# EPFL-VILAB/MultiMAE

Measured on AMD Instinct MI355X. Metric: pre-train images/sec (whole node), ViT-B RGB+D+S 224^2 98-vis-tok, higher is better.
Workload: dtype bf16 (fp32_output_adapters: fp16 storage); 1 GPU; BASELINE.json configs[2]: ViT-B, RGB+depth+semseg, 224^2, Dirichlet alpha=1.0, 98 visible tokens, 4 cross-attention decoders (dim 256, depth 2), semseg adapter (fp32_output_adapters) with fp16 STORAGE (activations / saved tensors / gradients of the adapter as IEEE half in HBM: every matmul input carries the 11-bit significand TF32 gave the reference on A100; gradients stored times a power of two f; per_gpu_batch=256, global_batch=256, parallelism=dp1

## Files before the change

include/mmae.h:

```cpp
#ifndef MMAE_H
#define MMAE_H

#include <stddef.h>
#include <stdint.h>

#ifdef __cplusplus
extern "C" {
#endif

#define MMAE_ABI_VERSION 7

#define MMAE_F32  0
#define MMAE_BF16 1
#define MMAE_F32X3 2
#define MMAE_F32F16 3
#define MMAE_MXFP8 4

#define MMAE_F16 5

#define MMAE_EINVAL   (-1)
#define MMAE_ELAUNCH  (-2)
#define MMAE_ESUPPORT (-3)

int mmae_abi_version(void);
// ... 27 lines not shown
    int32_t tile;
    int32_t split_k;
    void* ws;
    int64_t ws_elems;
    float* colsum_part;
    float* a_colsum;
    int32_t a_colsum_acc;
    const void* a_scale;
    const void* b_scale;
    void* q_out; void* q_scale;
    int64_t ldq;
    const float* a_amax;
    const float* ln_gamma; const float* ln_beta; void* ln_out; float* ln_mean; float* ln_rstd; float ln_eps;
} mmae_gemm_desc;

int mmae_gemm(const mmae_gemm_desc* d, void* stream);
int mmae_gemm_plan(const mmae_gemm_desc* d, int* tile, int* split_k);
int mmae_gemm_auto_splitk(int M, int N, int K, int ab_dtype);
int mmae_gemm_cu_reserve(int k);
int mmae_gemm_cu_share(int k);
int mmae_gemm_side_cus(int k);
#ifdef MMAE_EXPERIMENTS
int mmae_gemm_duo_occupancy(int tile);
#endif

int64_t mmae_mx_scale_bytes(int rows, int cols);
int mmae_mx_quant(const void* x, int x_dtype, int64_t ldx, int rows, int cols, void* q, int64_t ldq, void* scales, void* stream);
int mmae_mx_quant_t(const void* w, int w_dtype, int64_t ldw, int n, int k, void* q, int64_t ldq, void* scales, void* stream);
int mmae_mx_quant_rows_t(const void* x, int x_dtype, int64_t ldx, int M, int C, void* q, int64_t ldq, void* scales, void* stream);
int mmae_mx_wgrad(int on);
int mmae_gelu_grad_aux(int on);
int mmae_ln_fuse(int on);
int mmae_xattn_fuse(int on);
int mmae_mx_scale_clear(void* scales, int rows, int cols, void* stream);
int mmae_layernorm_fwd_mx(const float* x, const float* gamma, const float* beta, void* y_bf16, float* mean, float* rstd, int64_t R, int D,
                          float eps, void* q, void* scales, void* stream);
int mmae_attn_fwd_mx(const void* q, const void* k, const void* v, void* o, float* lse, int B, int H, int Nq, int Nk, int hd,
                     int64_t q_sb, int64_t q_sr, int64_t k_sb, int64_t k_sr, int64_t v_sb, int64_t v_sr, int64_t o_sb, int64_t o_sr,
                     float scale, void* mx_q, void* mx_scale, void* stream);
int mmae_attn_bwd_mx(const void* q, const void* k, const void* v, const void* o, const void* d_o, const float* lse, void* dq, void* dk,
                     void* dv, int B, int H, int Nq, int Nk, int hd, int64_t q_sb, int64_t q_sr, int64_t k_sb, int64_t k_sr, int64_t v_sb,
                     int64_t v_sr, int64_t o_sb, int64_t o_sr, int64_t dq_sb, int64_t dq_sr, int64_t dk_sb, int64_t dk_sr, int64_t dv_sb,
                     int64_t dv_sr, float scale, void* mx_q, void* mx_scale, void* stream);
int64_t mmae_mx_tmp_bytes(int rows, int cols);
int mmae_mx_prepare_weights(int n, const void* const* w, int w_dtype, const int32_t* n_out, const int32_t* k_in, void* const* dst, void* stream);
int mmae_probe_mx_mfma(const int32_t* a_64x8, const int32_t* b_64x8, const int32_t* scale_a_64, const int32_t* scale_b_64, int opsel_a, int opsel_b,
                       float* out_64x16, void* stream);

int mmae_gemm_timing_enable(int on);
int mmae_gemm_timing_read(double* ms3, double* flop3, int64_t* calls3);
int mmae_gemm_timing_read_bytes(double* bytes3);

typedef struct mmae_dw_problem {
    const void* dy; int64_t ldy;
    const void* x; int64_t ldx;
    float* dw; float* db;
    int32_t n_out, k_in;
} mmae_dw_problem;

typedef struct mmae_dw_group_desc {
    int32_t n, rows, ab_dtype, accumulate, split_k;
    mmae_dw_problem p[8];
    float* ws; int64_t ws_elems;
    const float* unscale;
} mmae_dw_group_desc;

// ... 338 lines not shown
```

multimae_amd/_lib.py:

```python
from __future__ import annotations

import ctypes
import os
import re
from typing import Dict, List, Tuple

_PKG = os.path.dirname(os.path.abspath(__file__))
HEADER = os.path.join(os.path.dirname(_PKG), 'include', 'mmae.h')
LIB_PATH = os.environ.get('MMAE_LIB') or os.path.join(_PKG, 'libmmae_hip.so')

F32, BF16, F32X3, F32F16 = 0, 1, 2, 3
MXFP8 = 4
F16 = 5
U16, I32 = 6, 7
EPI_NONE, EPI_GELU, EPI_DGELU, EPI_GELU_G, EPI_MUL = 0, 1, 2, 3, 4


class GemmDesc(ctypes.Structure):
    _fields_ = [
        ('A', ctypes.c_void_p), ('B', ctypes.c_void_p), ('C', ctypes.c_void_p),
        ('ab_dtype', ctypes.c_int32), ('c_dtype', ctypes.c_int32),
        ('M', ctypes.c_int32), ('N', ctypes.c_int32), ('K', ctypes.c_int32),
        ('a_trans', ctypes.c_int32), ('b_trans', ctypes.c_int32),
        ('lda', ctypes.c_int64), ('ldb', ctypes.c_int64), ('ldc', ctypes.c_int64),
# ... 123 lines not shown
_lib = None


def declared_symbols() -> List[str]:
    return sorted(_PROTOS)


def load() -> ctypes.CDLL:
    global _lib
    if _lib is not None:
        return _lib
    if not os.path.exists(LIB_PATH):
        raise RuntimeError(
            f'{LIB_PATH} not found: the MI355X kernel library is not built. '
            'Run `python -c "import __graft_entry__ as g; g.build()"` (or `make -C multimae_amd/csrc`). '
            'multimae_amd has no CPU / PyTorch fallback by design.')
    lib = ctypes.CDLL(LIB_PATH)
    for name, (ret, argtypes) in _PROTOS.items():
        fn = getattr(lib, name)
        fn.restype = ret
        fn.argtypes = argtypes
    if lib.mmae_abi_version() != 7:
        raise RuntimeError('libmmae_hip.so ABI version mismatch')
    for which, cls in enumerate((GemmDesc, BlockDesc, StackDesc, AdapterDesc, OptDesc, PatchSrc, DwGroupDesc, ColsumJob,
                                     OptGroupsDesc)):
        if lib.mmae_struct_size(which) != ctypes.sizeof(cls):
            raise RuntimeError(f'{cls.__name__}: ctypes mirror ({ctypes.sizeof(cls)} B) != library struct ({lib.mmae_struct_size(which)} B)')
    if os.environ.get('MMAE_MX_WGRAD') is not None:
        lib.mmae_mx_wgrad(int(os.environ['MMAE_MX_WGRAD'] != '0'))
    if os.environ.get('MMAE_LN_FUSE') is not None:
        lib.mmae_ln_fuse(int(os.environ['MMAE_LN_FUSE'] != '0'))
    if os.environ.get('MMAE_XATTN_FUSE') is not None:
        lib.mmae_xattn_fuse(int(os.environ['MMAE_XATTN_FUSE'] != '0'))
    if os.environ.get('MMAE_GELU_GRAD_AUX') is not None:
        lib.mmae_gelu_grad_aux(int(os.environ['MMAE_GELU_GRAD_AUX'] != '0'))
    _lib = lib
    return lib


class KernelError(RuntimeError):
    pass


def check(rc: int, what: str) -> None:
    if rc != 0:
        msg = load().mmae_last_error()
        raise KernelError(f'{what} failed (rc={rc}): {msg.decode() if msg else "?"}')
```

multimae_amd/csrc/attention.hip:

```cpp
#include "common.h"
#include <mutex>

#define LDS_AS __attribute__((address_space(3)))
typedef __attribute__((ext_vector_type(8))) short s16x8;

namespace {

constexpr unsigned OOB = 0x80000000u;

struct AttnArgs {
    const void *q, *k, *v, *o, *d_o;
    void *out, *dq, *dk, *dv;
    float* lse;
    int B, H, Nq, Nk, nqp, nkp;
    long long q_sb, q_sr, k_sb, k_sr, v_sb, v_sr, o_sb, o_sr, dq_sb, dq_sr, dk_sb, dk_sr, dv_sb, dv_sr;
    float scale;
    unsigned char *mx_q, *mx_s;
    long long mx_rows;
    int mx_ld, mx_col[3];
    const float* dy_amax;
};

template <int HD> __device__ __forceinline__ int tile_off(int row, int c);
template <> __device__ __forceinline__ int tile_off<64>(int row, int c) {
    return (row >> 1) * 256 + (((((row & 1) << 3) | c) ^ ((row >> 1) & 15)) << 4);
}
template <> __device__ __forceinline__ int tile_off<32>(int row, int c) {
    return (row >> 2) * 256 + (((((row & 3) << 2) | c) ^ ((row >> 2) & 15)) << 4);
}

template <int HD, int NTHR, int MAXR = 256>
struct TileLoader {
    static constexpr int CPR = HD / 8;
    static constexpr int MAXIT = (MAXR * CPR + NTHR - 1) / NTHR;
// ... 286 lines not shown
                l = lg;
            }
            m = mn;
#pragma unroll
            for (int t = 0; t < NT; ++t) {
                if (t0 + t < nt) {
#pragma unroll
                    for (int sI = 0; sI < 2; ++sI) {
                        const bf16x8 pf = pack8m<MODE>(s[t], sI);
                        const bf16x8 pl = X3 ? pack8_lo(s[t], sI) : pf;
#pragma unroll
                        for (int dt = 0; dt < HD / 32; ++dt) {
                            const bf16x8 vh = frag_cols<HD>(Vs, dt * 32, (t0 + t) * 32 + 16 * sI, lane);
                            const bf16x8 vl = X3 ? frag_cols<HD>(Vs + lo, dt * 32, (t0 + t) * 32 + 16 * sI, lane) : vh;
                            o[dt] = mma<MODE>(vh, vl, pf, pl, o[dt]);
                        }
                    }
                }
            }
        }
        {
            const float inv = 1.0f / l;
#pragma unroll
            for (int dt = 0; dt < HD / 32; ++dt) store_row32<MODE == 3>(ob + q * a.o_sr + dt * 32, o[dt], inv, hi, qok);
            if (MODE == 0 && a.mx_q) {
#pragma unroll
                for (int dt = 0; dt < HD / 32; ++dt) store_row32_mx(a, (long long)b * a.Nq + q, a.mx_col[0] + h * HD + dt * 32, o[dt], inv, hi, qok);
            }
            if (qok && hi == 0) a.lse[((long long)b * a.H + h) * a.Nq + q] = m * 0.69314718056f + __logf(l);
        }
    }
}

template <int HD, int MODE, int NW, bool RS = false>
__global__ void __launch_bounds__(NW * 64, NW == 4 ? 2 : 1) attn_bwd_kernel(const AttnArgs a) {
    static_assert(!RS || NW == 4, "register-resident pass 1: the passes run one after the other");
    constexpr int NTH = NW * 64;
    constexpr bool X3 = MODE == 1, F32IO = MODE == 1 || MODE == 2;
    typedef typename ActOf<F32IO>::T AT;
    float do_s = 1.0f, do_inv = 1.0f;
    if (MODE == 2 && a.dy_amax) {
        const unsigned e = (__float_as_uint(*a.dy_amax) >> 23) & 0xffu;
        if (e >= 1 && e <= 253) { do_s = __uint_as_float((254u - e) << 23); do_inv = __uint_as_float(e << 23); }
    }
    extern __shared__ __attribute__((aligned(16))) char smem[];
    const int tid = threadIdx.x, lane = tid & 63, hi = lane >> 5;
    const int wave = __builtin_amdgcn_readfirstlane(tid >> 6);
    const int b = blockIdx.x / a.H, h = blockIdx.x % a.H;
    char* Qs = smem;
    char* dOs = Qs + a.nqp * HD * 2;
    char* Ks = dOs + a.nqp * HD * 2;
    char* Vs = Ks + a.nkp * HD * 2;
    const int lo = 2 * (a.nqp + a.nkp) * HD * 2;
    float* lse_s = (float*)(Vs + a.nkp * HD * 2 + (X3 ? lo : 0));
    float* delta_s = lse_s + a.nqp;
    const AT* qg = (const AT*)a.q + b * a.q_sb + h * HD;
    const AT* dog = (const AT*)a.d_o + b * a.o_sb + h * HD;
    const AT* kg = (const AT*)a.k + b * a.k_sb + h * HD;
    const AT* vg = (const AT*)a.v + b * a.v_sb + h * HD;
    if constexpr (F32IO) {
        {
            TileLoaderF32<HD, NTH> lq, ld;
            lq.issue(qg, a.q_sr, a.Nq, a.nqp, tid);
            ld.issue(dog, a.o_sr, a.Nq, a.nqp, tid);
            for (int q = tid; q < a.nqp; q += NTH) lse_s[q] = q < a.Nq ? a.lse[((long long)b * a.H + h) * a.Nq + q] * 1.44269504089f : 0.f;
            if constexpr (X3) { lq.commit(Qs, lo, a.nqp, tid); ld.commit(dOs, lo, a.nqp, tid); }
            else { lq.commit16(Qs, a.nqp, tid, 1.0f); ld.commit16(dOs, a.nqp, tid, do_s); }
        }
        {
            TileLoaderF32<HD, NTH> lk, lv;
            lk.issue(kg, a.k_sr, a.Nk, a.nkp, tid);
            lv.issue(vg, a.v_sr, a.Nk, a.nkp, tid);
            if constexpr (X3) { lk.commit(Ks, lo, a.nkp, tid); lv.commit(Vs, lo, a.nkp, tid); }
            else { lk.commit16(Ks, a.nkp, tid, 1.0f); lv.commit16(Vs, a.nkp, tid, 1.0f); }
        }
    } else {
        TileLoader<HD, NTH> lq, ld, lk, lv;
        lq.issue(qg, a.q_sr, a.Nq, a.nqp, tid);
        ld.issue(dog, a.o_sr, a.Nq, a.nqp, tid);
        lk.issue(kg, a.k_sr, a.Nk, a.nkp, tid);
        lv.issue(vg, a.v_sr, a.Nk, a.nkp, tid);
        for (int q = tid; q < a.nqp; q += NTH) lse_s[q] = q < a.Nq ? a.lse[((long long)b * a.H + h) * a.Nq + q] * 1.44269504089f : 0.f;
        lq.commit(Qs, a.nqp, tid);
        ld.commit(dOs, a.nqp, tid);
        lk.commit(Ks, a.nkp, tid);
        lv.commit(Vs, a.nkp, tid);
    }
    const int nt = a.nkp >> 5, nqb = a.nqp >> 5;
    const float sc2 = a.scale * 1.44269504089f;
    __syncthreads();
    for (int qblk = wave; !RS && qblk < nqb; qblk += NW) {
        const int q = qblk * 32 + (lane & 31);
        bf16x8 qf[HD / 16], dof[HD / 16], ql[HD / 16], dol[HD / 16];
#pragma unroll
        for (int ks = 0; ks < HD / 16; ++ks) {
            qf[ks] = frag_rows<HD>(Qs, qblk * 32, ks, lane); dof[ks] = frag_rows<HD>(dOs, qblk * 32, ks, lane);
            ql[ks] = X3 ? frag_rows<HD>(Qs + lo, qblk * 32, ks, lane) : qf[ks];
            dol[ks] = X3 ? frag_rows<HD>(dOs + lo, qblk * 32, ks, lane) : dof[ks];
        }
        const float lse_q = lse_s[q];
        float d0 = 0.f, d1 = 0.f;
        for (int t = 0; t < nt; ++t) {
            f32x16 st, dpt;
#pragma unroll
            for (int r = 0; r < 16; ++r) { st[r] = 0.f; dpt[r] = 0.f; }
#pragma unroll
            for (int ks = 0; ks < HD / 16; ++ks) {
                const bf16x8 kh = frag_rows<HD>(Ks, t * 32, ks, lane), vh = frag_rows<HD>(Vs, t * 32, ks, lane);
                const bf16x8 kl = X3 ? frag_rows<HD>(Ks + lo, t * 32, ks, lane) : kh, vl = X3 ? frag_rows<HD>(Vs + lo, t * 32, ks, lane) : vh;
                st = mma<MODE>(kh, kl, qf[ks], ql[ks], st);
                dpt = mma<MODE>(vh, vl, dof[ks], dol[ks], dpt);
            }
#pragma unroll
            for (int r = 0; r < 16; r += 2) {
                d0 += __builtin_amdgcn_exp2f(st[r] * sc2 - lse_q) * dpt[r];
                d1 += __builtin_amdgcn_exp2f(st[r + 1] * sc2 - lse_q) * dpt[r + 1];
            }
        }
        float d = d0 + d1;
        d += __shfl_xor(d, 32, 64);
        if (hi == 0) delta_s[q] = d * a.scale;
    }
    if (!RS) __syncthreads();

    for (int qblk = wave; RS && qblk < nqb; qblk += 4) {
        const int q = qblk * 32 + (lane & 31);
        const bool qok = q < a.Nq;
        f32x16 st[4], dpt[4];
        {
            bf16x8 qf[HD / 16], dof[HD / 16];
#pragma unroll
            for (int ks = 0; ks < HD / 16; ++ks) { qf[ks] = frag_rows<HD>(Qs, qblk * 32, ks, lane); dof[ks] = frag_rows<HD>(dOs, qblk * 32, ks, lane); }
#pragma unroll
            for (int t = 0; t < 4; ++t) {
                if (t < nt) {
#pragma unroll
                    for (int r = 0; r < 16; ++r) { st[t][r] = 0.f; dpt[t][r] = 0.f; }
#pragma unroll
                    for (int ks = 0; ks < HD / 16; ++ks) {
                        const bf16x8 kh = frag_rows<HD>(Ks, t * 32, ks, lane), vh = frag_rows<HD>(Vs, t * 32, ks, lane);
                        st[t] = mma<MODE>(kh, kh, qf[ks], qf[ks], st[t]);
                        dpt[t] = mma<MODE>(vh, vh, dof[ks], dof[ks], dpt[t]);
                    }
                }
            }
        }
        const float lse_q = lse_s[q];
        float d0 = 0.f, d1 = 0.f;
#pragma unroll
        for (int t = 0; t < 4; ++t) {
            if (t < nt) {
#pragma unroll
                for (int r = 0; r < 16; r += 2) {
                    const float p0 = __builtin_amdgcn_exp2f(st[t][r] * sc2 - lse_q), p1 = __builtin_amdgcn_exp2f(st[t][r + 1] * sc2 - lse_q);
                    st[t][r] = p0; st[t][r + 1] = p1;
                    d0 += p0 * dpt[t][r]; d1 += p1 * dpt[t][r + 1];
                }
            }
        }
        float delta_q = d0 + d1;
        delta_q += __shfl_xor(delta_q, 32, 64);
        delta_q *= a.scale;
        if (hi == 0) delta_s[q] = delta_q;
        f32x16 dq[HD / 32];
#pragma unroll
        for (int dt = 0; dt < HD / 32; ++dt)
#pragma unroll
            for (int r = 0; r < 16; ++r) dq[dt][r] = 0.f;
#pragma unroll
        for (int t = 0; t < 4; ++t) {
            if (t < nt) {
#pragma unroll
                for (int r = 0; r < 16; ++r) st[t][r] = st[t][r] * (dpt[t][r] * a.scale - delta_q);
#pragma unroll
                for (int sI = 0; sI < 2; ++sI) {
                    const bf16x8 dsf = pack8m<MODE>(st[t], sI);
#pragma unroll
                    for (int dt = 0; dt < HD / 32; ++dt) {
                        const bf16x8 kh = frag_cols<HD>(Ks, dt * 32, t * 32 + 16 * sI, lane);
                        dq[dt] = mma<MODE>(kh, kh, dsf, dsf, dq[dt]);
                    }
                }
            }
        }
        AT* dst = (AT*)a.dq + b * a.dq_sb + h * HD + q * a.dq_sr;
#pragma unroll
        for (int dt = 0; dt < HD / 32; ++dt) store_row32<MODE == 3>(dst + dt * 32, dq[dt], do_inv, hi, qok);
        if (MODE == 0 && a.mx_q) {
#pragma unroll
            for (int dt = 0; dt < HD / 32; ++dt) store_row32_mx(a, (long long)b * a.Nq + q, a.mx_col[0] + h * HD + dt * 32, dq[dt], 1.0f, hi, qok);
        }
    }
    if (RS) __syncthreads();

    for (int qblk = wave; !RS && (NW == 4 || wave < 4) && qblk < nqb; qblk += 4) {
        const int q = qblk * 32 + (lane & 31);
        const bool qok = q < a.Nq;
        bf16x8 qf[HD / 16], dof[HD / 16], ql[HD / 16], dol[HD / 16];
#pragma unroll
        for (int ks = 0; ks < HD / 16; ++ks) {
            qf[ks] = frag_rows<HD>(Qs, qblk * 32, ks, lane); dof[ks] = frag_rows<HD>(dOs, qblk * 32, ks, lane);
            ql[ks] = X3 ? frag_rows<HD>(Qs + lo, qblk * 32, ks, lane) : qf[ks];
            dol[ks] = X3 ? frag_rows<HD>(dOs + lo, qblk * 32, ks, lane) : dof[ks];
        }
        const float lse_q = lse_s[q], delta_q = delta_s[q];
        f32x16 dq[HD / 32];
#pragma unroll
        for (int dt = 0; dt < HD / 32; ++dt)
#pragma unroll
            for (int r = 0; r < 16; ++r) dq[dt][r] = 0.f;
        for (int t = 0; t < nt; ++t) {
            f32x16 st, dpt;
#pragma unroll
            for (int r = 0; r < 16; ++r) { st[r] = 0.f; dpt[r] = 0.f; }
#pragma unroll
            for (int ks = 0; ks < HD / 16; ++ks) {
                const bf16x8 kh = frag_rows<HD>(Ks, t * 32, ks, lane), vh = frag_rows<HD>(Vs, t * 32, ks, lane);
                const bf16x8 kl = X3 ? frag_rows<HD>(Ks + lo, t * 32, ks, lane) : kh, vl = X3 ? frag_rows<HD>(Vs + lo, t * 32, ks, lane) : vh;
                st = mma<MODE>(kh, kl, qf[ks], ql[ks], st);
                dpt = mma<MODE>(vh, vl, dof[ks], dol[ks], dpt);
            }
#pragma unroll
            for (int r = 0; r < 16; ++r) {
                const float p = __builtin_amdgcn_exp2f(st[r] * sc2 - lse_q);
                st[r] = p * (dpt[r] * a.scale - delta_q);
            }
#pragma unroll
            for (int sI = 0; sI < 2; ++sI) {
                const bf16x8 dsf = pack8m<MODE>(st, sI);
                const bf16x8 dsl = X3 ? pack8_lo(st, sI) : dsf;
#pragma unroll
                for (int dt = 0; dt < HD / 32; ++dt) {
                    const bf16x8 kh = frag_cols<HD>(Ks, dt * 32, t * 32 + 16 * sI, lane);
                    const bf16x8 kl = X3 ? frag_cols<HD>(Ks + lo, dt * 32, t * 32 + 16 * sI, lane) : kh;
                    dq[dt] = mma<MODE>(kh, kl, dsf, dsl, dq[dt]);
                }
            }
        }
        {
            AT* dst = (AT*)a.dq + b * a.dq_sb + h * HD + q * a.dq_sr;
#pragma unroll
            for (int dt = 0; dt < HD / 32; ++dt) store_row32<MODE == 3>(dst + dt * 32, dq[dt], do_inv, hi, qok);
            if (MODE == 0 && a.mx_q) {
#pragma unroll
                for (int dt = 0; dt < HD / 32; ++dt) store_row32_mx(a, (long long)b * a.Nq + q, a.mx_col[0] + h * HD + dt * 32, dq[dt], 1.0f, hi, qok);
            }
        }
    }

    for (int kblk = (NW == 8 ? wave - 4 : wave); (NW == 4 || wave >= 4) && kblk < nt; kblk += 4) {
        const int key = kblk * 32 + (lane & 31);
        bf16x8 kf[HD / 16], vf[HD / 16], kl[HD / 16], vl[HD / 16];
#pragma unroll
        for (int ks = 0; ks < HD / 16; ++ks) {
            kf[ks] = frag_rows<HD>(Ks, kblk * 32, ks, lane); vf[ks] = frag_rows<HD>(Vs, kblk * 32, ks, lane);
            kl[ks] = X3 ? frag_rows<HD>(Ks + lo, kblk * 32, ks, lane) : kf[ks];
            vl[ks] = X3 ? frag_rows<HD>(Vs + lo, kblk * 32, ks, lane) : vf[ks];
        }
        f32x16 dk[HD / 32], dv[HD / 32];
#pragma unroll
        for (int dt = 0; dt < HD / 32; ++dt)
#pragma unroll
            for (int r = 0; r < 16; ++r) { dk[dt][r] = 0.f; dv[dt][r] = 0.f; }
        for (int qt = 0; qt < nqb; ++qt) {
            f32x16 sm, dp;
#pragma unroll
            for (int r = 0; r < 16; ++r) { sm[r] = 0.f; dp[r] = 0.f; }
#pragma unroll
            for (int ks = 0; ks < HD / 16; ++ks) {
                const bf16x8 qh = frag_rows<HD>(Qs, qt * 32, ks, lane), doh = frag_rows<HD>(dOs, qt * 32, ks, lane);
                const bf16x8 qlo = X3 ? frag_rows<HD>(Qs + lo, qt * 32, ks, lane) : qh, dolo = X3 ? frag_rows<HD>(dOs + lo, qt * 32, ks, lane) : doh;
                sm = mma<MODE>(qh, qlo, kf[ks], kl[ks], sm);
                dp = mma<MODE>(doh, dolo, vf[ks], vl[ks], dp);
            }
#pragma unroll
            for (int r = 0; r < 16; ++r) {
                const int qr = qt * 32 + (r & 3) + 8 * (r >> 2) + 4 * hi;
                const float p = __builtin_amdgcn_exp2f(sm[r] * sc2 - lse_s[qr]);
                sm[r] = p;
                dp[r] = p * (dp[r] * a.scale - delta_s[qr]);
            }
#pragma unroll
            for (int sI = 0; sI < 2; ++sI) {
                const bf16x8 pf = pack8m<MODE>(sm, sI), dsf = pack8m<MODE>(dp, sI);
                const bf16x8 pl = X3 ? pack8_lo(sm, sI) : pf, dsl = X3 ? pack8_lo(dp, sI) : dsf;
#pragma unroll
                for (int dt = 0; dt < HD / 32; ++dt) {
                    const bf16x8 doh = frag_cols<HD>(dOs, dt * 32, qt * 32 + 16 * sI, lane), qh = frag_cols<HD>(Qs, dt * 32, qt * 32 + 16 * sI, lane);
                    const bf16x8 dolo = X3 ? frag_cols<HD>(dOs + lo, dt * 32, qt * 32 + 16 * sI, lane) : doh;
                    const bf16x8 qlo = X3 ? frag_cols<HD>(Qs + lo, dt * 32, qt * 32 + 16 * sI, lane) : qh;
                    dv[dt] = mma<MODE>(doh, dolo, pf, pl, dv[dt]);
                    dk[dt] = mma<MODE>(qh, qlo, dsf, dsl, dk[dt]);
                }
            }
        }
        {
            const bool kok = key < a.Nk;
            AT* dkd = (AT*)a.dk + b * a.dk_sb + h * HD + key * a.dk_sr;
            AT* dvd = (AT*)a.dv + b * a.dv_sb + h * HD + key * a.dv_sr;
#pragma unroll
            for (int dt = 0; dt < HD / 32; ++dt) {
                store_row32<MODE == 3>(dkd + dt * 32, dk[dt], do_inv, hi, kok);
                store_row32<MODE == 3>(dvd + dt * 32, dv[dt], do_inv, hi, kok);
            }
            if (MODE == 0 && a.mx_q) {
#pragma unroll
                for (int dt = 0; dt < HD / 32; ++dt) {
                    store_row32_mx(a, (long long)b * a.Nk + key, a.mx_col[1] + h * HD + dt * 32, dk[dt], 1.0f, hi, kok);
                    store_row32_mx(a, (long long)b * a.Nk + key, a.mx_col[2] + h * HD + dt * 32, dv[dt], 1.0f, hi, kok);
                }
            }
        }
    }
}


struct XAttnArgs {
    const uint16_t *qn, *cn, *wq, *wkv;
    const float *bq, *bkv;
    uint16_t *q, *kv, *out;
    float* lse;
    int B, H, Nq, Nk;
    float scale;
};
__device__ __forceinline__ int xa_coff(int row, int ch) { return row * 512 + ((ch ^ (row & 31)) << 4); }
__device__ __forceinline__ int xa_dperm(int i) { return (i & ~12) | ((i & 4) << 1) | ((i & 8) >> 1); }

__global__ void __launch_bounds__(256, 2) xattn_fwd_fused_kernel(const XAttnArgs a) {
    constexpr int D = 256, HD = 32, NT = 4, KS = D / 16;
    extern __shared__ __attribute__((aligned(16))) char smem[];
    const int tid = threadIdx.x, lane = tid & 63, hi = lane >> 5;
    const int wave = __builtin_amdgcn_readfirstlane(tid >> 6);
    const int b = blockIdx.x / a.H, h = blockIdx.x % a.H;
    char* Cs = smem;
    char* Ks = smem;
    char* Vs = smem + 128 * HD * 2;
    {
        const auto rsC = __builtin_amdgcn_make_buffer_rsrc((void*)(a.cn + (long long)b * a.Nk * D), 0, 0x80000000, 0x00020000);
        i32x4 r[16];
#pragma unroll
        for (int i = 0; i < 16; ++i) {
            const int c = tid + i * 256, row = c >> 5, ch = c & 31;
            r[i] = __builtin_amdgcn_raw_buffer_load_b128(rsC, row < a.Nk ? (unsigned)((row * D + ch * 8) * 2) : OOB, 0, 0);
        }
#pragma unroll
        for (int i = 0; i < 16; ++i) {
// ... 461 lines not shown
    a.q = q; a.k = k; a.v = v; a.out = o; a.lse = lse;
    a.B = B; a.H = H; a.Nq = Nq; a.Nk = Nk; a.nqp = (Nq + 31) / 32 * 32; a.nkp = (Nk + 31) / 32 * 32;
    a.q_sb = q_sb; a.q_sr = q_sr; a.k_sb = k_sb; a.k_sr = k_sr; a.v_sb = v_sb; a.v_sr = v_sr; a.o_sb = o_sb; a.o_sr = o_sr;
    a.scale = scale;
    if (mx_q) {
        MMAE_REQUIRE(!x3 && mx_scale && o_sr == (int64_t)H * hd && o_sb == (int64_t)Nq * o_sr, "attn_fwd_mx: bf16 output, dense [B * Nq][H * head_dim]");
        a.mx_q = (unsigned char*)mx_q; a.mx_s = (unsigned char*)mx_scale; a.mx_rows = (long long)B * Nq; a.mx_ld = H * hd;
    }
    const size_t lds = (size_t)2 * a.nkp * hd * 2 * (x3 ? 2 : 1);
    hipStream_t st_ = (hipStream_t)stream;
    dim3 grid(B * H), block(256);
#define LAUNCH_FWD(HD, NT, X3, ...)                                                                                                       \
    do {                                                                                                                                  \
        hipFuncSetAttribute((const void*)attn_fwd_kernel<HD, NT, X3, ##__VA_ARGS__>, hipFuncAttributeMaxDynamicSharedMemorySize, (int)lds); \
        hipLaunchKernelGGL((attn_fwd_kernel<HD, NT, X3, ##__VA_ARGS__>), grid, block, lds, st_, a);                                         \
    } while (0)
    static const int env_grp = mmae_env_int("MMAE_ATTN_FWD_GRP", 1);
    const bool small = a.nkp <= 128, mid = a.nkp <= 224;
    if (mode == 1) {
        if (hd == 64) { if (small) LAUNCH_FWD(64, 4, 1); else if (mid) LAUNCH_FWD(64, 7, 1); else LAUNCH_FWD(64, 8, 1); }
        else { if (small) LAUNCH_FWD(32, 4, 1); else if (mid) LAUNCH_FWD(32, 7, 1); else LAUNCH_FWD(32, 8, 1); }
    } else if (mode == 2) {
        if (hd == 64) { if (small) LAUNCH_FWD(64, 4, 2); else if (mid) LAUNCH_FWD(64, 7, 2); else LAUNCH_FWD(64, 8, 2); }
        else { if (small) LAUNCH_FWD(32, 4, 2); else if (mid) LAUNCH_FWD(32, 7, 2); else LAUNCH_FWD(32, 8, 2); }
    } else if (mode == 3) {
        if (hd == 64) { if (small) LAUNCH_FWD(64, 4, 3); else if (mid) LAUNCH_FWD(64, 7, 3); else LAUNCH_FWD(64, 8, 3); }
        else { if (small) LAUNCH_FWD(32, 4, 3); else if (env_grp) LAUNCH_FWD(32, 4, 3, true); else if (mid) LAUNCH_FWD(32, 7, 3); else LAUNCH_FWD(32, 8, 3); }
    } else {
        if (hd == 64) { if (small) LAUNCH_FWD(64, 4, 0); else if (mid) LAUNCH_FWD(64, 7, 0); else LAUNCH_FWD(64, 8, 0); }
        else { if (small) LAUNCH_FWD(32, 4, 0); else if (env_grp) LAUNCH_FWD(32, 4, 0, true); else if (mid) LAUNCH_FWD(32, 7, 0); else LAUNCH_FWD(32, 8, 0); }
    }
#undef LAUNCH_FWD
    return mmae_check_launch("attn_fwd");
}

static int attn_bwd_impl(int mode, const void* q, const void* k, const void* v, const void* o, const void* d_o, const float* lse, void* dq,
                         void* dk, void* dv, int B, int H, int Nq, int Nk, int hd, int64_t q_sb, int64_t q_sr, int64_t k_sb, int64_t k_sr,
                         int64_t v_sb, int64_t v_sr, int64_t o_sb, int64_t o_sr, int64_t dq_sb, int64_t dq_sr, int64_t dk_sb, int64_t dk_sr,
                         int64_t dv_sb, int64_t dv_sr, float scale, void* stream, void* mx_q = nullptr, void* mx_scale = nullptr,
                         const float* dy_amax = nullptr) {
    const bool x3 = mode == 1;
    MMAE_REQUIRE(q && k && v && o && d_o && lse && dq && dk && dv, "attn_bwd: null pointer");
    MMAE_REQUIRE(((uintptr_t)dq % 16 == 0) && ((uintptr_t)dk % 16 == 0) && ((uintptr_t)dv % 16 == 0), "attn_bwd: unaligned output pointer");
    const long long st[] = {q_sb, q_sr, k_sb, k_sr, v_sb, v_sr, o_sb, o_sr, dq_sb, dq_sr, dk_sb, dk_sr, dv_sb, dv_sr};
    const int rc = check_common(B, H, Nq, Nk, hd, st, 14);
    MMAE_REQUIRE(rc == 0, rc == -2 ? "attn: head_dim must be 32 or 64" : (rc == -3 ? "attn: strides must be multiples of 8" : "attn: need 1 <= Nq, Nk <= 256"));
    AttnArgs a = {};
    a.q = q; a.k = k; a.v = v; a.o = o; a.d_o = d_o;
    a.dq = dq; a.dk = dk; a.dv = dv; a.lse = (float*)lse;
    a.B = B; a.H = H; a.Nq = Nq; a.Nk = Nk; a.nqp = (Nq + 31) / 32 * 32; a.nkp = (Nk + 31) / 32 * 32;
    a.q_sb = q_sb; a.q_sr = q_sr; a.k_sb = k_sb; a.k_sr = k_sr; a.v_sb = v_sb; a.v_sr = v_sr; a.o_sb = o_sb; a.o_sr = o_sr;
    a.dq_sb = dq_sb; a.dq_sr = dq_sr; a.dk_sb = dk_sb; a.dk_sr = dk_sr; a.dv_sb = dv_sb; a.dv_sr = dv_sr;
    a.scale = scale;
    a.dy_amax = dy_amax;
    if (mx_q) {
        const int64_t Dm = (int64_t)H * hd;
        MMAE_REQUIRE(!x3 && mx_scale && Nq == Nk && dq_sr == 3 * Dm && dk_sr == 3 * Dm && dv_sr == 3 * Dm && dq_sb == Nq * 3 * Dm && dk_sb == dq_sb && dv_sb == dq_sb &&
                     (const uint16_t*)dk == (const uint16_t*)dq + Dm && (const uint16_t*)dv == (const uint16_t*)dq + 2 * Dm,
                     "attn_bwd_mx: dq, dk, dv must be the column slices of one packed bf16 [B * N][3 D] tensor");
        a.mx_q = (unsigned char*)mx_q; a.mx_s = (unsigned char*)mx_scale; a.mx_rows = (long long)B * Nq; a.mx_ld = (int)(3 * Dm);
        a.mx_col[0] = 0; a.mx_col[1] = (int)Dm; a.mx_col[2] = (int)(2 * Dm);
    }
    const size_t lds = (size_t)2 * (a.nqp + a.nkp) * hd * 2 * (x3 ? 2 : 1) + (size_t)2 * a.nqp * 4;
    if (lds > 160 * 1024) { mmae_set_error("attn_bwd: tiles exceed the 160 KB LDS (f32 split path: (Nq + Nk) * head_dim too large)"); return MMAE_ESUPPORT; }
    hipStream_t st_ = (hipStream_t)stream;
    dim3 grid(B * H);
#define LAUNCH_BWD(HD, X3, NW, ...)                                                                                                       \
    do {                                                                                                                                  \
        hipFuncSetAttribute((const void*)attn_bwd_kernel<HD, X3, NW, ##__VA_ARGS__>, hipFuncAttributeMaxDynamicSharedMemorySize, (int)lds); \
        hipLaunchKernelGGL((attn_bwd_kernel<HD, X3, NW, ##__VA_ARGS__>), grid, dim3(NW * 64), lds, st_, a);                                 \
    } while (0)
    static const int env_rs = mmae_env_int("MMAE_ATTN_BWD_RS", 1);
    const bool rs = env_rs && a.nkp <= 128 && lds <= 80 * 1024;
    if (mode == 1) { if (hd == 64) LAUNCH_BWD(64, 1, 8); else LAUNCH_BWD(32, 1, 8); }
    else if (mode == 2) { if (hd == 64) { if (lds <= 80 * 1024) LAUNCH_BWD(64, 2, 4); else LAUNCH_BWD(64, 2, 8); } else LAUNCH_BWD(32, 2, 8); }
    else if (mode == 3) { if (hd == 64) { if (lds <= 80 * 1024) LAUNCH_BWD(64, 3, 4); else LAUNCH_BWD(64, 3, 8); } else if (rs) LAUNCH_BWD(32, 3, 4, true); else LAUNCH_BWD(32, 3, 8); }
    else if (hd == 64) { if (rs) LAUNCH_BWD(64, 0, 4, true); else if (lds <= 80 * 1024) LAUNCH_BWD(64, 0, 4); else LAUNCH_BWD(64, 0, 8); }
    else {
        static const int env_rs32 = mmae_env_int("MMAE_ATTN_BWD_RS32", 1);
        if (rs && env_rs32) LAUNCH_BWD(32, 0, 4, true); else LAUNCH_BWD(32, 0, 8);
    }
#undef LAUNCH_BWD
    return mmae_check_launch("attn_bwd");
}


int mmae_xattn_fwd_fused(const void* qn, const void* cn, const void* wq, const float* bq, const void* wkv, const float* bkv, void* q, void* kv,
                         void* out, float* lse, int B, int H, int Nq, int Nk, int D, float scale, void* stream) {
    MMAE_REQUIRE(qn && cn && wq && bq && wkv && bkv && q && kv && out && lse, "xattn_fwd_fused: null pointer");
    if (D != 256 || H != 8 || Nk < 1 || Nk > 128 || Nq < 1 || B < 1) { mmae_set_error("xattn_fwd_fused: D = 8 x 32 = 256 and 1 <= Nk <= 128 only"); return MMAE_ESUPPORT; }
    MMAE_REQUIRE(((uintptr_t)qn | (uintptr_t)cn | (uintptr_t)wq | (uintptr_t)wkv | (uintptr_t)q | (uintptr_t)kv | (uintptr_t)out | (uintptr_t)bq | (uintptr_t)bkv) % 16 == 0,
                 "xattn_fwd_fused: unaligned pointer");
    XAttnArgs a = {(const uint16_t*)qn, (const uint16_t*)cn, (const uint16_t*)wq, (const uint16_t*)wkv, bq, bkv, (uint16_t*)q, (uint16_t*)kv, (uint16_t*)out, lse,
                   B, H, Nq, Nk, scale};
    const size_t lds = (size_t)128 * 256 * 2;
    static std::once_flag once;
    std::call_once(once, [&] { (void)hipFuncSetAttribute((const void*)xattn_fwd_fused_kernel, hipFuncAttributeMaxDynamicSharedMemorySize, (int)lds); });
    hipLaunchKernelGGL(xattn_fwd_fused_kernel, dim3(B * H), dim3(256), lds, (hipStream_t)stream, a);
    return mmae_check_launch("xattn_fwd_fused");
}

int mmae_attn_fwd(const void* q, const void* k, const void* v, void* o, float* lse, int B, int H, int Nq, int Nk, int hd,
                  int64_t q_sb, int64_t q_sr, int64_t k_sb, int64_t k_sr, int64_t v_sb, int64_t v_sr, int64_t o_sb, int64_t o_sr,
                  float scale, void* stream) {
    return attn_fwd_impl(0, q, k, v, o, lse, B, H, Nq, Nk, hd, q_sb, q_sr, k_sb, k_sr, v_sb, v_sr, o_sb, o_sr, scale, stream);
}
int mmae_attn_fwd_mx(const void* q, const void* k, const void* v, void* o, float* lse, int B, int H, int Nq, int Nk, int hd,
                     int64_t q_sb, int64_t q_sr, int64_t k_sb, int64_t k_sr, int64_t v_sb, int64_t v_sr, int64_t o_sb, int64_t o_sr,
                     float scale, void* mx_q, void* mx_scale, void* stream) {
    MMAE_REQUIRE(mx_q && mx_scale, "attn_fwd_mx: null MX destination");
    return attn_fwd_impl(0, q, k, v, o, lse, B, H, Nq, Nk, hd, q_sb, q_sr, k_sb, k_sr, v_sb, v_sr, o_sb, o_sr, scale, stream, mx_q, mx_scale);
}
int mmae_attn_fwd_f32x3(const void* q, const void* k, const void* v, void* o, float* lse, int B, int H, int Nq, int Nk, int hd,
                        int64_t q_sb, int64_t q_sr, int64_t k_sb, int64_t k_sr, int64_t v_sb, int64_t v_sr, int64_t o_sb, int64_t o_sr,
                        float scale, void* stream) {
// ... 114 lines not shown
```

multimae_amd/ops.py:

```python
from __future__ import annotations

import ctypes
import math
from typing import Optional, Sequence

import torch

from . import _lib
import contextlib

from ._lib import BF16, F16, F32, F32X3, F32F16, MXFP8, EPI_NONE, EPI_GELU, EPI_DGELU, EPI_GELU_G, EPI_MUL, AdapterDesc, BlockDesc, DwGroupDesc, GemmDesc, OptDesc, OptGroupsDesc, PatchSrc, StackDesc, check

Tensor = torch.Tensor


def _require_gpu(t: Tensor, name: str = 'tensor') -> None:
    if not t.is_cuda:
        raise RuntimeError(f'multimae_amd: {name} is on {t.device}; the engine runs on MI355X HIP kernels only '
                           '(no CPU / PyTorch fallback). Move the model and inputs to a GPU.')


def dcode(dtype: torch.dtype) -> int:
    if dtype == torch.float32:
        return F32
# ... 181 lines not shown
    d.A, d.B, d.C = a.q.data_ptr(), b.q.data_ptr(), C.data_ptr()
    d.a_scale, d.b_scale = a.scales.data_ptr(), b.scales.data_ptr()
    d.ab_dtype, d.c_dtype = MXFP8, dcode(C.dtype)
    d.M, d.N, d.K = M, N, K
    d.lda, d.ldb, d.ldc = K, K, N
    d.batch = d.batch_inner = 1
    d.bias = _p(bias)
    d.resid, d.ldr = _p(resid), N
    d.aux, d.ldaux = _p(aux), N
    d.aux_dtype = dcode(aux.dtype) if aux is not None else F32
    d.epi, d.alpha, d.split_k = epi, 1.0, split_k
    d.accumulate = int(accumulate)
    if split_k > 1:
        ws = stream_workspace(_stream(), C.device, max(_WS_ELEMS[0], split_k * M * N))
        d.ws, d.ws_elems = ws.data_ptr(), ws.numel()
    d.colsum_part = _p(colsum_part)
    if q_out is not None:
        assert q_out.rows == M and q_out.cols == N
        d.q_out, d.q_scale, d.ldq = q_out.q.data_ptr(), q_out.scales.data_ptr(), N
    check(_lib.load().mmae_gemm(ctypes.byref(d), _stream()), 'mmae_gemm(mxfp8)')
    return C


def gemm_cu_reserve(k: Optional[int] = None) -> int:
    return int(_lib.load().mmae_gemm_cu_reserve(-1 if k is None else int(k)))


def ln_fuse(on: Optional[bool] = None) -> bool:
    return bool(_lib.load().mmae_ln_fuse(-1 if on is None else int(bool(on))))


def xattn_fuse(on: Optional[bool] = None) -> bool:
    return bool(_lib.load().mmae_xattn_fuse(-1 if on is None else int(bool(on))))


def gemm_cu_share(k: Optional[int] = None) -> int:
    return int(_lib.load().mmae_gemm_cu_share(-1 if k is None else int(k)))


def gemm_side_cus(k: Optional[int] = None) -> int:
    return int(_lib.load().mmae_gemm_side_cus(-1 if k is None else int(k)))


def linear_fwd(x: Tensor, w: Tensor, bias: Optional[Tensor], out: Tensor, *, resid: Optional[Tensor] = None,
               aux: Optional[Tensor] = None, epi: int = EPI_NONE, tile: int = 0, ln: Optional[tuple] = None) -> Tensor:
    M, K = x.shape
    N = w.shape[0]
    gemm(x, w, out, M, N, K, lda=K, ldb=K, ldc=N, bias=bias, resid=resid, ldr=N, aux=aux, ldaux=N, epi=epi, tile=tile, ln=ln)
    return out


def linear_dx(dy: Tensor, w: Tensor, out: Tensor, *, aux: Optional[Tensor] = None, epi: int = EPI_NONE,
              colsum_out: Optional[Tensor] = None, colsum_part: Optional[Tensor] = None, tile: int = 0) -> Tensor:
    M, N = dy.shape
    K = w.shape[1]
    part = colsum_part
    if colsum_out is not None and part is None:
        part = torch.empty(dx_colsum_part_shape(M, K), device=dy.device, dtype=torch.float32)
    gemm(dy, w, out, M, K, N, lda=dy.stride(0), ldb=K, ldc=K, b_trans=True, aux=aux, ldaux=K, epi=epi, colsum_part=part, tile=tile)
    if colsum_out is not None:
        colsum(part, colsum_out, False)
    return out


def gemm_dw_group(problems: Sequence[tuple], accumulate: bool, split_k: int = 0, unscale: Optional[Tensor] = None) -> None:
    d = DwGroupDesc()
# ... 1193 lines not shown
```

Before: 8928 images/s.

## Make attention backward persistent and prefetch next head's tiles during last key pass

The attention backward kernel now loops over heads with a grid capped at twice the CU count, enabled by default. During the last key-block pass it issues global loads for the next head's K/V, Q/dO and LSE, hiding load latency behind MFMA work. The MX-fp8 mirror store becomes a template parameter, so the runtime branch drops out of non-MX variants. This adds register pressure and extra syncs, and can cost load balance compared with one block per head.

```diff
diff --git a/include/mmae.h b/include/mmae.h
--- a/include/mmae.h
+++ b/include/mmae.h
@@ -83,6 +83,8 @@
 int mmae_gelu_grad_aux(int on);
 int mmae_ln_fuse(int on);
 int mmae_xattn_fuse(int on);
+int mmae_attn_bwd_persist(int on);
+int mmae_attn_bwd_persist_grid(int max_grid);
 int mmae_mx_scale_clear(void* scales, int rows, int cols, void* stream);
 int mmae_layernorm_fwd_mx(const float* x, const float* gamma, const float* beta, void* y_bf16, float* mean, float* rstd, int64_t R, int D,
                           float eps, void* q, void* scales, void* stream);
diff --git a/multimae_amd/_lib.py b/multimae_amd/_lib.py
--- a/multimae_amd/_lib.py
+++ b/multimae_amd/_lib.py
@@ -179,6 +179,8 @@
         lib.mmae_ln_fuse(int(os.environ['MMAE_LN_FUSE'] != '0'))
     if os.environ.get('MMAE_XATTN_FUSE') is not None:
         lib.mmae_xattn_fuse(int(os.environ['MMAE_XATTN_FUSE'] != '0'))
+    if os.environ.get('MMAE_ATTN_BWD_PERSIST') is not None:
+        lib.mmae_attn_bwd_persist(int(os.environ['MMAE_ATTN_BWD_PERSIST'] != '0'))
     if os.environ.get('MMAE_GELU_GRAD_AUX') is not None:
         lib.mmae_gelu_grad_aux(int(os.environ['MMAE_GELU_GRAD_AUX'] != '0'))
     _lib = lib
diff --git a/multimae_amd/csrc/attention.hip b/multimae_amd/csrc/attention.hip
--- a/multimae_amd/csrc/attention.hip
+++ b/multimae_amd/csrc/attention.hip
@@ -1,5 +1,8 @@
 #include "common.h"
+#include <algorithm>
+#include <atomic>
 #include <mutex>
+#include <type_traits>
 
 #define LDS_AS __attribute__((address_space(3)))
 typedef __attribute__((ext_vector_type(8))) short s16x8;
@@ -352,11 +355,14 @@
     }
 }
 
-template <int HD, int MODE, int NW, bool RS = false>
+template <int HD, int MODE, int NW, bool RS = false, bool MX = false>
 __global__ void __launch_bounds__(NW * 64, NW == 4 ? 2 : 1) attn_bwd_kernel(const AttnArgs a) {
     static_assert(!RS || NW == 4, "register-resident pass 1: the passes run one after the other");
+    static_assert(!MX || MODE == 0, "the MX-fp8 mirror accompanies bf16 outputs");
     constexpr int NTH = NW * 64;
     constexpr bool X3 = MODE == 1, F32IO = MODE == 1 || MODE == 2;
+    constexpr bool PF = NW == 4 && !F32IO;
+    constexpr int KR = RS ? 128 : 256;
     typedef typename ActOf<F32IO>::T AT;
     float do_s = 1.0f, do_inv = 1.0f;
     if (MODE == 2 && a.dy_amax) {
@@ -364,9 +370,6 @@
         if (e >= 1 && e <= 253) { do_s = __uint_as_float((254u - e) << 23); do_inv = __uint_as_float(e << 23); }
     }
     extern __shared__ __attribute__((aligned(16))) char smem[];
-    const int tid = threadIdx.x, lane = tid & 63, hi = lane >> 5;
-    const int wave = __builtin_amdgcn_readfirstlane(tid >> 6);
-    const int b = blockIdx.x / a.H, h = blockIdx.x % a.H;
     char* Qs = smem;
     char* dOs = Qs + a.nqp * HD * 2;
     char* Ks = dOs + a.nqp * HD * 2;
@@ -374,10 +377,20 @@
     const int lo = 2 * (a.nqp + a.nkp) * HD * 2;
     float* lse_s = (float*)(Vs + a.nkp * HD * 2 + (X3 ? lo : 0));
     float* delta_s = lse_s + a.nqp;
+    const int nt = a.nkp >> 5, nqb = a.nqp >> 5, nheads = a.B * a.H;
+    const float sc2 = a.scale * 1.44269504089f;
+  for (int head = blockIdx.x;; head += gridDim.x) {
+    int tid = threadIdx.x;
+    if constexpr (PF) asm volatile("" : "+v"(tid));
+    const int lane = tid & 63, hi = lane >> 5;
+    const int wave = __builtin_amdgcn_readfirstlane(tid >> 6);
+    const int b = head / a.H, h = head % a.H;
+    const bool more = PF && head + (int)gridDim.x < nheads;
     const AT* qg = (const AT*)a.q + b * a.q_sb + h * HD;
     const AT* dog = (const AT*)a.d_o + b * a.o_sb + h * HD;
     const AT* kg = (const AT*)a.k + b * a.k_sb + h * HD;
     const AT* vg = (const AT*)a.v + b * a.v_sb + h * HD;
+    float lse_n = 0.f;
     if constexpr (F32IO) {
         {
             TileLoaderF32<HD, NTH> lq, ld;
@@ -394,8 +407,9 @@
             if constexpr (X3) { lk.commit(Ks, lo, a.nkp, tid); lv.commit(Vs, lo, a.nkp, tid); }
             else { lk.commit16(Ks, a.nkp, tid, 1.0f); lv.commit16(Vs, a.nkp, tid, 1.0f); }
         }
-    } else {
-        TileLoader<HD, NTH> lq, ld, lk, lv;
+    } else if (!PF || head == (int)blockIdx.x) {
+        TileLoader<HD, NTH> lq, ld;
+        TileLoader<HD, NTH, KR> lk, lv;
         lq.issue(qg, a.q_sr, a.Nq, a.nqp, tid);
         ld.issue(dog, a.o_sr, a.Nq, a.nqp, tid);
         lk.issue(kg, a.k_sr, a.Nk, a.nkp, tid);
@@ -406,8 +420,6 @@
         lk.commit(Ks, a.nkp, tid);
         lv.commit(Vs, a.nkp, tid);
     }
-    const int nt = a.nkp >> 5, nqb = a.nqp >> 5;
-    const float sc2 = a.scale * 1.44269504089f;
     __syncthreads();
     for (int qblk = wave; !RS && qblk < nqb; qblk += NW) {
         const int q = qblk * 32 + (lane & 31);
@@ -453,9 +465,9 @@
             for (int ks = 0; ks < HD / 16; ++ks) { qf[ks] = frag_rows<HD>(Qs, qblk * 32, ks, lane); dof[ks] = frag_rows<HD>(dOs, qblk * 32, ks, lane); }
 #pragma unroll
             for (int t = 0; t < 4; ++t) {
+#pragma unroll
+                for (int r = 0; r < 16; ++r) { st[t][r] = 0.f; dpt[t][r] = 0.f; }
                 if (t < nt) {
-#pragma unroll
-                    for (int r = 0; r < 16; ++r) { st[t][r] = 0.f; dpt[t][r] = 0.f; }
 #pragma unroll
                     for (int ks = 0; ks < HD / 16; ++ks) {
                         const bf16x8 kh = frag_rows<HD>(Ks, t * 32, ks, lane), vh = frag_rows<HD>(Vs, t * 32, ks, lane);
@@ -506,7 +518,7 @@
         AT* dst = (AT*)a.dq + b * a.dq_sb + h * HD + q * a.dq_sr;
 #pragma unroll
         for (int dt = 0; dt < HD / 32; ++dt) store_row32<MODE == 3>(dst + dt * 32, dq[dt], do_inv, hi, qok);
-        if (MODE == 0 && a.mx_q) {
+        if constexpr (MX) {
 #pragma unroll
             for (int dt = 0; dt < HD / 32; ++dt) store_row32_mx(a, (long long)b * a.Nq + q, a.mx_col[0] + h * HD + dt * 32, dq[dt], 1.0f, hi, qok);
         }
@@ -561,28 +573,40 @@
             AT* dst = (AT*)a.dq + b * a.dq_sb + h * HD + q * a.dq_sr;
 #pragma unroll
             for (int dt = 0; dt < HD / 32; ++dt) store_row32<MODE == 3>(dst + dt * 32, dq[dt], do_inv, hi, qok);
-            if (MODE == 0 && a.mx_q) {
+            if constexpr (MX) {
 #pragma unroll
                 for (int dt = 0; dt < HD / 32; ++dt) store_row32_mx(a, (long long)b * a.Nq + q, a.mx_col[0] + h * HD + dt * 32, dq[dt], 1.0f, hi, qok);
             }
         }
     }
 
-    for (int kblk = (NW == 8 ? wave - 4 : wave); (NW == 4 || wave >= 4) && kblk < nt; kblk += 4) {
+  {
+    int tid = threadIdx.x;
+    if constexpr (PF) asm volatile("" : "+v"(tid));
+    const int lane = tid & 63, hi = lane >> 5;
+    const int nb = (head + (int)gridDim.x) / a.H, nh = (head + (int)gridDim.x) % a.H;
+    constexpr int QR = HD == 64 ? 128 : 256;
+    const bool qpre = a.nqp <= QR;
+    TileLoader<HD, NTH, QR> pq, pd;
+    auto kpass = [&](const int kblk, const bool act, auto last_c) {
+        constexpr bool LAST = decltype(last_c)::value;
         const int key = kblk * 32 + (lane & 31);
-        bf16x8 kf[HD / 16], vf[HD / 16], kl[HD / 16], vl[HD / 16];
-#pragma unroll
-        for (int ks = 0; ks < HD / 16; ++ks) {
-            kf[ks] = frag_rows<HD>(Ks, kblk * 32, ks, lane); vf[ks] = frag_rows<HD>(Vs, kblk * 32, ks, lane);
-            kl[ks] = X3 ? frag_rows<HD>(Ks + lo, kblk * 32, ks, lane) : kf[ks];
-            vl[ks] = X3 ? frag_rows<HD>(Vs + lo, kblk * 32, ks, lane) : vf[ks];
-        }
+        bf16x8 kf[HD / 16] = {}, vf[HD / 16] = {}, kl[HD / 16] = {}, vl[HD / 16] = {};
         f32x16 dk[HD / 32], dv[HD / 32];
 #pragma unroll
         for (int dt = 0; dt < HD / 32; ++dt)
 #pragma unroll
             for (int r = 0; r < 16; ++r) { dk[dt][r] = 0.f; dv[dt][r] = 0.f; }
-        for (int qt = 0; qt < nqb; ++qt) {
+        if (act) {
+#pragma unroll
+            for (int ks = 0; ks < HD / 16; ++ks) {
+                kf[ks] = frag_rows<HD>(Ks, kblk * 32, ks, lane); vf[ks] = frag_rows<HD>(Vs, kblk * 32, ks, lane);
+                kl[ks] = X3 ? frag_rows<HD>(Ks + lo, kblk * 32, ks, lane) : kf[ks];
+                vl[ks] = X3 ? frag_rows<HD>(Vs + lo, kblk * 32, ks, lane) : vf[ks];
+            }
+        }
+        auto qstep = [&](const int qt) {
+            if (!act) return;
             f32x16 sm, dp;
 #pragma unroll
             for (int r = 0; r < 16; ++r) { sm[r] = 0.f; dp[r] = 0.f; }
@@ -613,8 +637,29 @@
                     dk[dt] = mma<MODE>(qh, qlo, dsf, dsl, dk[dt]);
                 }
             }
-        }
-        {
+        };
+        if constexpr (PF && LAST) {
+            TileLoader<HD, NTH, KR> pk, pv;
+            if (more) {
+                __syncthreads();
+                pk.issue((const uint16_t*)a.k + nb * a.k_sb + nh * HD, a.k_sr, a.Nk, a.nkp, tid);
+                pv.issue((const uint16_t*)a.v + nb * a.v_sb + nh * HD, a.v_sr, a.Nk, a.nkp, tid);
+            }
+            qstep(0);
+            if (more) {
+                pk.commit(Ks, a.nkp, tid);
+                pv.commit(Vs, a.nkp, tid);
+                if (qpre) {
+                    pq.issue((const uint16_t*)a.q + nb * a.q_sb + nh * HD, a.q_sr, a.Nq, a.nqp, tid);
+                    pd.issue((const uint16_t*)a.d_o + nb * a.o_sb + nh * HD, a.o_sr, a.Nq, a.nqp, tid);
+                }
+                if (tid < a.Nq) lse_n = a.lse[((long long)nb * a.H + nh) * a.Nq + tid] * 1.44269504089f;
+            }
+            for (int qt = 1; qt < nqb; ++qt) qstep(qt);
+        } else {
+            for (int qt = 0; qt < nqb; ++qt) qstep(qt);
+        }
+        if (act) {
             const bool kok = key < a.Nk;
             AT* dkd = (AT*)a.dk + b * a.dk_sb + h * HD + key * a.dk_sr;
             AT* dvd = (AT*)a.dv + b * a.dv_sb + h * HD + key * a.dv_sr;
@@ -623,7 +668,7 @@
                 store_row32<MODE == 3>(dkd + dt * 32, dk[dt], do_inv, hi, kok);
                 store_row32<MODE == 3>(dvd + dt * 32, dv[dt], do_inv, hi, kok);
             }
-            if (MODE == 0 && a.mx_q) {
+            if constexpr (MX) {
 #pragma unroll
                 for (int dt = 0; dt < HD / 32; ++dt) {
                     store_row32_mx(a, (long long)b * a.Nk + key, a.mx_col[1] + h * HD + dt * 32, dk[dt], 1.0f, hi, kok);
@@ -631,7 +676,31 @@
                 }
             }
         }
-    }
+    };
+    if constexpr (PF) {
+        int kb0 = 0;
+        if constexpr (!RS)
+            for (; kb0 + 4 < nt; kb0 += 4) kpass(kb0 + wave, true, std::false_type());
+        kpass(kb0 + wave, kb0 + wave < nt, std::true_type());
+        if (!more) break;
+        __syncthreads();
+        if (qpre) {
+            pq.commit(Qs, a.nqp, tid);
+            pd.commit(dOs, a.nqp, tid);
+        } else {
+            TileLoader<HD, NTH> fq, fd;
+            fq.issue((const AT*)a.q + nb * a.q_sb + nh * HD, a.q_sr, a.Nq, a.nqp, tid);
+            fd.issue((const AT*)a.d_o + nb * a.o_sb + nh * HD, a.o_sr, a.Nq, a.nqp, tid);
+            fq.commit(Qs, a.nqp, tid);
+            fd.commit(dOs, a.nqp, tid);
+        }
+        if (tid < a.nqp) lse_s[tid] = lse_n;
+    } else {
+        for (int kblk = (NW == 8 ? wave - 4 : wave); (NW == 4 || wave >= 4) && kblk < nt; kblk += 4) kpass(kblk, true, std::false_type());
+        break;
+    }
+  }
+  }
 }
 
 
@@ -1159,6 +1228,18 @@
     }
 #undef LAUNCH_FWD
     return mmae_check_launch("attn_fwd");
+}
+
+std::atomic<int> g_attn_bwd_persist{1}, g_attn_bwd_grid{0};
+int mmae_attn_bwd_persist(int on) {
+    const int prev = g_attn_bwd_persist.load(std::memory_order_relaxed);
+    if (on >= 0) g_attn_bwd_persist.store(on ? 1 : 0, std::memory_order_relaxed);
+    return prev;
+}
+int mmae_attn_bwd_persist_grid(int max_grid) {
+    const int prev = g_attn_bwd_grid.load(std::memory_order_relaxed);
+    if (max_grid >= 0) g_attn_bwd_grid.store(max_grid, std::memory_order_relaxed);
+    return prev;
 }
 
 static int attn_bwd_impl(int mode, const void* q, const void* k, const void* v, const void* o, const void* d_o, const float* lse, void* dq,
@@ -1191,23 +1272,33 @@
     const size_t lds = (size_t)2 * (a.nqp + a.nkp) * hd * 2 * (x3 ? 2 : 1) + (size_t)2 * a.nqp * 4;
     if (lds > 160 * 1024) { mmae_set_error("attn_bwd: tiles exceed the 160 KB LDS (f32 split path: (Nq + Nk) * head_dim too large)"); return MMAE_ESUPPORT; }
     hipStream_t st_ = (hipStream_t)stream;
-    dim3 grid(B * H);
-#define LAUNCH_BWD(HD, X3, NW, ...)                                                                                                       \
+    int pgrid = B * H;
+    if (g_attn_bwd_persist.load(std::memory_order_relaxed)) {
+        const int cap = g_attn_bwd_grid.load(std::memory_order_relaxed);
+        pgrid = std::min(pgrid, cap > 0 ? cap : 2 * mmae_cu_count());
+    }
+#define LAUNCH_BWD_(HD, X3, NW, RS, MX)                                                                                                   \
     do {                                                                                                                                  \
-        hipFuncSetAttribute((const void*)attn_bwd_kernel<HD, X3, NW, ##__VA_ARGS__>, hipFuncAttributeMaxDynamicSharedMemorySize, (int)lds); \
-        hipLaunchKernelGGL((attn_bwd_kernel<HD, X3, NW, ##__VA_ARGS__>), grid, dim3(NW * 64), lds, st_, a);                                 \
+        const dim3 grid((NW == 4 && (X3 == 0 || X3 == 3)) ? pgrid : B * H);                                                               \
+        hipFuncSetAttribute((const void*)attn_bwd_kernel<HD, X3, NW, RS, MX>, hipFuncAttributeMaxDynamicSharedMemorySize, (int)lds);       \
+        hipLaunchKernelGGL((attn_bwd_kernel<HD, X3, NW, RS, MX>), grid, dim3(NW * 64), lds, st_, a);                                      \
+    } while (0)
+#define LAUNCH_BWD(HD, X3, NW, RS)                                                                                                        \
+    do {                                                                                                                                  \
+        if (X3 == 0 && a.mx_q) LAUNCH_BWD_(HD, X3, NW, RS, (X3 == 0)); else LAUNCH_BWD_(HD, X3, NW, RS, false);                            \
     } while (0)
     static const int env_rs = mmae_env_int("MMAE_ATTN_BWD_RS", 1);
     const bool rs = env_rs && a.nkp <= 128 && lds <= 80 * 1024;
-    if (mode == 1) { if (hd == 64) LAUNCH_BWD(64, 1, 8); else LAUNCH_BWD(32, 1, 8); }
-    else if (mode == 2) { if (hd == 64) { if (lds <= 80 * 1024) LAUNCH_BWD(64, 2, 4); else LAUNCH_BWD(64, 2, 8); } else LAUNCH_BWD(32, 2, 8); }
-    else if (mode == 3) { if (hd == 64) { if (lds <= 80 * 1024) LAUNCH_BWD(64, 3, 4); else LAUNCH_BWD(64, 3, 8); } else if (rs) LAUNCH_BWD(32, 3, 4, true); else LAUNCH_BWD(32, 3, 8); }
-    else if (hd == 64) { if (rs) LAUNCH_BWD(64, 0, 4, true); else if (lds <= 80 * 1024) LAUNCH_BWD(64, 0, 4); else LAUNCH_BWD(64, 0, 8); }
+    if (mode == 1) { if (hd == 64) LAUNCH_BWD(64, 1, 8, false); else LAUNCH_BWD(32, 1, 8, false); }
+    else if (mode == 2) { if (hd == 64) { if (lds <= 80 * 1024) LAUNCH_BWD(64, 2, 4, false); else LAUNCH_BWD(64, 2, 8, false); } else LAUNCH_BWD(32, 2, 8, false); }
+    else if (mode == 3) { if (hd == 64) { if (lds <= 80 * 1024) LAUNCH_BWD(64, 3, 4, false); else LAUNCH_BWD(64, 3, 8, false); } else if (rs) LAUNCH_BWD(32, 3, 4, true); else LAUNCH_BWD(32, 3, 8, false); }
+    else if (hd == 64) { if (rs) LAUNCH_BWD(64, 0, 4, true); else if (lds <= 80 * 1024) LAUNCH_BWD(64, 0, 4, false); else LAUNCH_BWD(64, 0, 8, false); }
     else {
         static const int env_rs32 = mmae_env_int("MMAE_ATTN_BWD_RS32", 1);
-        if (rs && env_rs32) LAUNCH_BWD(32, 0, 4, true); else LAUNCH_BWD(32, 0, 8);
+        if (rs && env_rs32) LAUNCH_BWD(32, 0, 4, true); else LAUNCH_BWD(32, 0, 8, false);
     }
 #undef LAUNCH_BWD
+#undef LAUNCH_BWD_
     return mmae_check_launch("attn_bwd");
 }
 
diff --git a/multimae_amd/ops.py b/multimae_amd/ops.py
--- a/multimae_amd/ops.py
+++ b/multimae_amd/ops.py
@@ -237,6 +237,14 @@
 
 def xattn_fuse(on: Optional[bool] = None) -> bool:
     return bool(_lib.load().mmae_xattn_fuse(-1 if on is None else int(bool(on))))
+
+
+def attn_bwd_persist(on: Optional[bool] = None) -> bool:
+    return bool(_lib.load().mmae_attn_bwd_persist(-1 if on is None else int(bool(on))))
+
+
+def attn_bwd_persist_grid(max_grid: Optional[int] = None) -> int:
+    return int(_lib.load().mmae_attn_bwd_persist_grid(-1 if max_grid is None else int(max_grid)))
 
 
 def gemm_cu_share(k: Optional[int] = None) -> int:
```

After: 8908 images/s. About the same (-0.2%).
